# travelingspaceman/LowThrustOpt

Measured on NVIDIA B200. Metric: segment-propagations/s (fp64 state+STM), higher is better.
Workload: dtype f64

## Files before the change

lowthrustopt_b200/csrc/lto_direct_cw.cu:

```cuda
#include "lto_internal.h"
#include "lto_cw_common.cuh"
#include <algorithm>

namespace lto {

namespace cw {

constexpr int NTILE = 2;
constexpr int NSLOT = 2;
constexpr int XW0 = 2;

template <int NS>
struct Cfg {
    static constexpr int NCOL = NS + 3;
    static constexpr int NW = NTILE + NCOL;
    static constexpr int NTHREADS = 32 * NW;
    static constexpr int SVAL = (NS == 7) ? 10 : 6;
    static constexpr int OFF_H = 13 * SVAL;
    static constexpr int OFF_BM = OFF_H + 1;
    static constexpr int STEP_DOUBLES = OFF_BM + ((NS == 7) ? 3 : 0);
    static constexpr size_t REC_BYTES = (size_t)NTILE * NSLOT * STEP_DOUBLES * 32 * sizeof(double);
    static constexpr int NV = 2 * (NS + 3);
    static constexpr size_t OUT_TILE_BYTES = (size_t)16 * NS * NV * sizeof(double);
    static constexpr size_t OUT_BYTES = (size_t)NTILE * OUT_TILE_BYTES;
    static constexpr size_t BAR_OFF = REC_BYTES + OUT_BYTES;
    static constexpr size_t FLAG_OFF = BAR_OFF + (size_t)NTILE * NSLOT * 2 * sizeof(unsigned long long);
    static constexpr size_t SMEM = FLAG_OFF + (size_t)NTILE * NSLOT * sizeof(int);
};

using namespace cwc;

template <int NS, bool PUB = true>
__device__ __forceinline__ double x_step(double (&r)[3], double (&v)[3], double& m, const double (&u)[3], double omega,
                                         double mdot, double h, const EPConst& c, double* __restrict__ rec, double& maxErr) {
    constexpr int SVAL = Cfg<NS>::SVAL;
    const double h2 = h * h;
    const double w2 = 2.0 * omega;
    const double kom6 = c.kthr / c.default_mass;
    double a[13][3];
    double ev[3] = {0.0, 0.0, 0.0}, ea[3] = {0.0, 0.0, 0.0};
    if (PUB) rec[Cfg<NS>::OFF_H * 32] = h;
#pragma unroll
    for (int j = 0; j < 13; ++j) {
        double R[3], V[3];
#pragma unroll
        for (int q = 0; q < 3; ++q) {
            double accv = 0.0, accr = 0.0;
#pragma unroll
            for (int l = 0; l < j; ++l) {
                if (lto_tab::Bf(j, l) != 0.0) accv = fma(lto_tab::Bf(j, l), a[l][q], accv);
                if (lto_tab::Gf(j, l) != 0.0) accr = fma(lto_tab::Gf(j, l), a[l][q], accr);
            }
            V[q] = (j == 0) ? v[q] : fma(h, accv, v[q]);
            R[q] = (j == 0) ? r[q] : fma(h2, accr, fma(h * lto_tab::Cf(j), v[q], r[q]));
        }
        const double dx1 = R[0] + c.mu, dx2 = dx1 - 1.0;
        const double yz = fma(R[1], R[1], R[2] * R[2]);
        const double i1 = fast_rsqrt(fma(dx1, dx1, yz));
        const double i2 = fast_rsqrt(fma(dx2, dx2, yz));
        const double i1s = i1 * i1, i2s = i2 * i2;
        const double a31 = c.m1 * i1s * i1, a32 = c.mu * i2s * i2;
        const double gg1 = 1.0 - (a31 + a32);
        double kom = kom6, im = 0.0;
        if (NS == 7) { im = fast_rcp(fma(h * lto_tab::Cf(j), mdot, m)); kom = c.kthr * im; }
        a[j][0] = fma(u[0], kom, fma(-a31, dx1, fma(-a32, dx2, fma(w2, V[1], R[0]))));
        a[j][1] = fma(u[1], kom, fma(gg1, R[1], -w2 * V[0]));
        a[j][2] = fma(u[2], kom, (gg1 - 1.0) * R[2]);
        if (PUB && j != 10) {
            const double a51 = 3.0 * i1s * a31, a52 = 3.0 * i2s * a32;
            const double s5 = a51 + a52;
            const double p1 = a51 * dx1, p2 = a52 * dx2;
            const double t = p1 + p2;
            const double s5y = s5 * R[1];
            double* w = rec + j * SVAL * 32;
            w[0 * 32] = fma(p1, dx1, fma(p2, dx2, gg1));
            w[1 * 32] = fma(s5y, R[1], gg1);
            w[2 * 32] = fma(s5 * R[2], R[2], gg1 - 1.0);
            w[3 * 32] = t * R[1];
            w[4 * 32] = t * R[2];
            w[5 * 32] = s5y * R[2];
            if (NS == 7) {
                w[6 * 32] = kom;
                const double k2 = -kom * im;
#pragma unroll
                for (int q = 0; q < 3; ++q) w[(7 + q) * 32] = k2 * u[q];
            }
        }
        if (lto_tab::PSIf(j) != 0.0) {
#pragma unroll
            for (int q = 0; q < 3; ++q) { ev[q] = fma(lto_tab::PSIf(j), V[q], ev[q]); ea[q] = fma(lto_tab::PSIf(j), a[j][q], ea[q]); }
        }
    }
    double delta = 0.0;
#pragma unroll
    for (int q = 0; q < 3; ++q) {
        double sv = 0.0, sr = 0.0;
#pragma unroll
        for (int l = 0; l < 13; ++l) {
            if (lto_tab::CHIf(l) != 0.0) sv = fma(lto_tab::CHIf(l), a[l][q], sv);
            if (lto_tab::CHIBf(l) != 0.0) sr = fma(lto_tab::CHIBf(l), a[l][q], sr);
        }
        r[q] = fma(h2, sr, fma(h, v[q], r[q]));
        v[q] = fma(h, sv, v[q]);
        delta = fmax(delta, fmax(fabs(ev[q]), fabs(ea[q])));
    }
    if (NS == 7) m = fma(h, mdot, m);
    delta *= fabs(h * lto_tab::ERRC);
    maxErr = fmax(maxErr, delta);
    return delta;
}

template <int NS>
__device__ __forceinline__ void col_step(double (&sr)[3], double (&sv)[3], double& sm, double bm, const double (&ec)[3],
                                         double omega, double kom6, const double* __restrict__ rec) {
    constexpr int SVAL = Cfg<NS>::SVAL;
    constexpr bool MASS = (NS == 7);
    const double h = rec[Cfg<NS>::OFF_H * 32];
    const double h2 = h * h;
    const double w2 = 2.0 * omega;
    double a[13][3];
#pragma unroll
    for (int j = 0; j < 13; ++j) {
        if (j == 10) continue;
        double R[3], V[3];
#pragma unroll
        for (int q = 0; q < 3; ++q) {
            double accv = 0.0, accr = 0.0;
#pragma unroll
            for (int l = 0; l < j; ++l) {
                if (lto_tab::Bf(j, l) != 0.0) accv = fma(lto_tab::Bf(j, l), a[l][q], accv);
                if (lto_tab::Gf(j, l) != 0.0) accr = fma(lto_tab::Gf(j, l), a[l][q], accr);
            }
            V[q] = (j == 0) ? sv[q] : fma(h, accv, sv[q]);
            R[q] = (j == 0) ? sr[q] : fma(h2, accr, fma(h * lto_tab::Cf(j), sv[q], sr[q]));
        }
        const double* w = rec + j * SVAL * 32;
        double U[6];
#pragma unroll
        for (int q = 0; q < 6; ++q) U[q] = w[q * 32];
        const double kom = MASS ? w[6 * 32] : kom6;
        double acc[3];
        acc[0] = fma(ec[0], kom, w2 * V[1]);
        acc[1] = fma(ec[1], kom, -w2 * V[0]);
        acc[2] = ec[2] * kom;
        if (MASS) {
            const double smj = fma(h * lto_tab::Cf(j), bm, sm);
#pragma unroll
            for (int q = 0; q < 3; ++q) acc[q] = fma(w[(7 + q) * 32], smj, acc[q]);
        }
        sym3_mul_acc(U, R, acc);
#pragma unroll
        for (int q = 0; q < 3; ++q) a[j][q] = acc[q];
    }
#pragma unroll
    for (int q = 0; q < 3; ++q) {
        double dv = 0.0, dr = 0.0;
#pragma unroll
        for (int l = 0; l < 13; ++l) {
            if (lto_tab::CHIf(l) != 0.0) dv = fma(lto_tab::CHIf(l), a[l][q], dv);
            if (lto_tab::CHIBf(l) != 0.0) dr = fma(lto_tab::CHIBf(l), a[l][q], dr);
        }
        sr[q] = fma(h2, dr, fma(h, sv[q], sr[q]));
        sv[q] = fma(h, dv, sv[q]);
    }
    if (MASS) sm = fma(h, bm, sm);
}

struct ColState { double sr[3], sv[3], sm, bm; };

template <int NS>
__device__ __forceinline__ void col_init(ColState& c, int col) {
#pragma unroll
    for (int q = 0; q < 3; ++q) { c.sr[q] = (col == q) ? 1.0 : 0.0; c.sv[q] = (col == q + 3) ? 1.0 : 0.0; }
    c.sm = (NS == 7 && col == 6) ? 1.0 : 0.0;
    c.bm = 0.0;
}

template <int NS>
__device__ __forceinline__ void col_store(double* __restrict__ stage, const ColState& c, int col, int lane) {
    constexpr int NV = 2 * (NS + 3);
    const int back = lane & 1, gc = col - NS;
    const int ocol = (gc >= 0) ? (2 * NS + (back ? 3 : 0) + gc) : ((back ? NS : 0) + col);
    double* J = stage + (lane >> 1) * (NS * NV) + ocol * NS;
    const double rj = (col >= 3 && col < 6) ? -1.0 : 1.0;
    const double sp = back ? -rj : 1.0;
    const double sq = back ? rj : 1.0;
    J[0] = sp * c.sr[0]; J[1] = sp * c.sr[1]; J[2] = sp * c.sr[2];
    J[3] = sq * c.sv[0]; J[4] = sq * c.sv[1]; J[5] = sq * c.sv[2];
    if (NS == 7) J[6] = sp * c.sm;
}

template <int NS>
__device__ __forceinline__ void column_warp(const DirectArgs& a, long long n_tiles, int col, int lane, double* recs, double* outs, unsigned bars) {
    typedef Cfg<NS> C;
    const int nstep = a.cfg.nsteps - 1;
    const double omega = (lane & 1) ? -1.0 : 1.0;
    const double kom6 = a.c.kthr / a.c.default_mass;
    const int gc = col - NS;
    const double ec[3] = {gc == 0 ? 1.0 : 0.0, gc == 1 ? 1.0 : 0.0, gc == 2 ? 1.0 : 0.0};
    ColState cs[NTILE];
    unsigned g = 0;
    for (long long pair = blockIdx.x; pair * NTILE < n_tiles; pair += gridDim.x) {
#pragma unroll
        for (int t = 0; t < NTILE; ++t) col_init<NS>(cs[t], col);
        for (int k = 0; k < nstep; ++k, ++g) {
            const unsigned slot = g & (NSLOT - 1), par = (g / NSLOT) & 1;
#ifndef LTO_K1_NO_PACE
            asm volatile("bar.sync 3, %0;" ::"n"(32 * C::NCOL) : "memory");
#endif
#pragma unroll
            for (int t = 0; t < NTILE; ++t) {
                const double* rec = recs + (size_t)(t * NSLOT + slot) * C::STEP_DOUBLES * 32 + lane;
                const unsigned full = bars + (unsigned)((t * NSLOT + slot) * 16), empty = full + 8;
                mbar_wait(full, par);
                if (NS == 7 && k == 0 && gc >= 0) cs[t].bm = rec[(C::OFF_BM + gc) * 32];
                col_step<NS>(cs[t].sr, cs[t].sv, cs[t].sm, cs[t].bm, ec, omega, kom6, rec);
                mbar_arrive(empty);
                if (k == nstep - 1) {
                    const long long tile = pair * NTILE + t;
                    const long long seg0 = tile * 16;
                    double* stage = outs + (size_t)t * (C::OUT_TILE_BYTES / sizeof(double));
                    const bool leader = (col == 0 && lane == 0);
                    if (leader) bulk_store_wait_read_but<NTILE - 1>();
                    asm volatile("bar.sync 2, %0;" ::"n"(32 * C::NCOL) : "memory");
                    col_store<NS>(stage, cs[t], col, lane);
                    fence_proxy_async();
                    asm volatile("bar.sync 2, %0;" ::"n"(32 * C::NCOL) : "memory");
                    if (leader && seg0 < a.n_seg) {
                        const long long nseg = (a.n_seg - seg0 < 16) ? (a.n_seg - seg0) : 16;
                        bulk_store(a.jac + seg0 * (long long)(NS * C::NV), smem_u32(stage), (unsigned)(nseg * NS * C::NV * sizeof(double)));
                    }
                }
            }
        }
    }
    if (col == 0 && lane == 0) bulk_store_wait_all();
}

template <int NS>
__device__ __forceinline__ void state_warp(const DirectArgs& a, long long n_tiles, int t, int lane, double* recs, unsigned bars) {
    typedef Cfg<NS> C;
    const int nsteps = a.cfg.nsteps, nstep = nsteps - 1;
    const int back = lane & 1;
    const double omega = back ? -1.0 : 1.0;
    double r[3], v[3], m = a.c.default_mass, u[3], bm[3] = {0.0, 0.0, 0.0}, mdot = 0.0, t0 = 0.0, t1 = 1.0, maxErr = 0.0;
    unsigned g = 0;
    for (long long pair = blockIdx.x; pair * NTILE < n_tiles; pair += gridDim.x) {
        const long long seg = (pair * NTILE + t) * 16 + (lane >> 1);
        {
            const long long sc = seg < a.n_seg ? seg : a.n_seg - 1;
            const long long ia = lto_node_a(sc, a.npt);
            const double* X = (back ? a.Xb : a.Xa) + ia * NS;
            const double* U = (back ? a.ub : a.ua) + ia * 3;
            r[0] = X[0]; r[1] = X[1]; r[2] = X[2];
            v[0] = X[3]; v[1] = X[4]; v[2] = X[5];
            if (back) { v[0] = -v[0]; v[1] = -v[1]; v[2] = -v[2]; }
            if (NS == 7) m = X[6];
            u[0] = U[0]; u[1] = U[1]; u[2] = U[2];
            const double ta = a.ta[ia], tb = a.tb[ia];
            t0 = ta; t1 = ta + (tb - ta) / 2.0;
            const double un = sqrt(fma(u[0], u[0], fma(u[1], u[1], u[2] * u[2])));
            mdot = -omega * un * a.c.cmdot;
            if (NS == 7) {
#pragma unroll
                for (int q = 0; q < 3; ++q) {
                    const double uh = (un > 0.0) ? u[q] / un : 1.0;
                    bm[q] = -omega * a.c.cmdot * uh;
                }
            }
            maxErr = 0.0;
        }
        for (int k = 0; k < nstep; ++k, ++g) {
            const unsigned slot = g & (NSLOT - 1), use = g / NSLOT;
            double* rec = recs + (size_t)(t * NSLOT + slot) * C::STEP_DOUBLES * 32 + lane;
            const unsigned full = bars + (unsigned)((t * NSLOT + slot) * 16), empty = full + 8;
            if (use > 0) mbar_wait(empty, (use - 1) & 1);
            const double h = linrange_at(t0, t1, nsteps, k + 1) - linrange_at(t0, t1, nsteps, k);
            if (NS == 7) {
#pragma unroll
                for (int q = 0; q < 3; ++q) rec[(C::OFF_BM + q) * 32] = bm[q];
            }
            x_step<NS>(r, v, m, u, omega, mdot, h, a.c, rec, maxErr);
            mbar_arrive(full);
        }
        const unsigned fullmask = 0xffffffffu;
        double xe[NS];
        xe[0] = r[0]; xe[1] = r[1]; xe[2] = r[2];
        xe[3] = back ? -v[0] : v[0]; xe[4] = back ? -v[1] : v[1]; xe[5] = back ? -v[2] : v[2];
        if (NS == 7) xe[6] = m;
        bool bad = false;
#pragma unroll
        for (int q = 0; q < NS; ++q) {
            const double other = __shfl_xor_sync(fullmask, xe[q], 1);
            const double d = xe[q] - other;
            bad |= !(d == d);
            if (!back && seg < a.n_seg) a.defect[seg * NS + q] = d;
        }
        const double me_o = __shfl_xor_sync(fullmask, maxErr, 1);
        if (!back && seg < a.n_seg) {
            if (a.errors) a.errors[seg] = fmax(maxErr, me_o);
            if (a.status) a.status[seg] = bad ? LTO_ST_NAN : LTO_OK;
        }
    }
}


template <int NS>
__device__ __forceinline__ void state_warp_adapt(const DirectArgs& a, long long n_tiles, int t, int lane, double* recs, unsigned bars, volatile int* lastf) {
    typedef Cfg<NS> C;
    const int back = lane & 1;
    const double omega = back ? -1.0 : 1.0;
    const unsigned fullmask = 0xffffffffu;
    double r[3], v[3], m = a.c.default_mass, u[3], bm[3] = {0.0, 0.0, 0.0}, mdot = 0.0, dummy = 0.0;
    unsigned g = 0;
    for (long long pair = blockIdx.x; pair * NTILE < n_tiles; pair += gridDim.x) {
        const long long seg = (pair * NTILE + t) * 16 + (lane >> 1);
        const long long sc = seg < a.n_seg ? seg : a.n_seg - 1;
        const long long ia = lto_node_a(sc, a.npt);
        const double* X = (back ? a.Xb : a.Xa) + ia * NS;
        const double* U = (back ? a.ub : a.ua) + ia * 3;
        r[0] = X[0]; r[1] = X[1]; r[2] = X[2];
        v[0] = X[3]; v[1] = X[4]; v[2] = X[5];
        if (back) { v[0] = -v[0]; v[1] = -v[1]; v[2] = -v[2]; }
        if (NS == 7) m = X[6];
        u[0] = U[0]; u[1] = U[1]; u[2] = U[2];
        const double ta = a.ta[ia], tb = a.tb[ia];
        const double t0 = ta, tfinal = ta + (tb - ta) / 2.0;
        const double un = sqrt(fma(u[0], u[0], fma(u[1], u[1], u[2] * u[2])));
        mdot = -omega * un * a.c.cmdot;
        if (NS == 7) {
#pragma unroll
            for (int q = 0; q < 3; ++q) { const double uh = (un > 0.0) ? u[q] / un : 1.0; bm[q] = -omega * a.c.cmdot * uh; }
        }
        const double hmax = (tfinal - t0) / 2.5, hmin = (tfinal - t0) / 1e7;
        double tt = t0, h = (tfinal - t0) / 50.0;
        int status = 0, nt = 0;
        bool done = !((tt < tfinal) && (h >= hmin));
        while (true) {
            const unsigned slot = g & (NSLOT - 1), use = g / NSLOT;
            double* rec = recs + (size_t)(t * NSLOT + slot) * C::STEP_DOUBLES * 32 + lane;
            const unsigned full = bars + (unsigned)((t * NSLOT + slot) * 16), empty = full + 8;
            if (use > 0) mbar_wait(empty, (use - 1) & 1);
            if (NS == 7) {
#pragma unroll
                for (int q = 0; q < 3; ++q) rec[(C::OFF_BM + q) * 32] = bm[q];
            }
            bool pending = !done;
            if (done) {
#pragma unroll
                for (int j = 0; j < 13 * C::SVAL; ++j) rec[j * 32] = 0.0;
                rec[C::OFF_H * 32] = 0.0;
            }
            while (__any_sync(fullmask, pending)) {
                if (pending) {
                    if (tt + h > tfinal) h = tfinal - tt;
                    if (nt >= a.cfg.max_attempts) { status = LTO_ST_MAXSTEPS; done = true; pending = false; }
                }
                if (pending) {
                    ++nt;
                    double r2[3] = {r[0], r[1], r[2]}, v2[3] = {v[0], v[1], v[2]}, m2 = m;
                    const double xn = fmax(fmax(fmax(fabs(r[0]), fabs(r[1])), fmax(fabs(r[2]), fabs(v[0]))), fmax(fmax(fabs(v[1]), fabs(v[2])), NS == 7 ? fabs(m) : 0.0));
                    double delta = x_step<NS>(r2, v2, m2, u, omega, mdot, h, a.c, rec, dummy);
                    if (!(delta == delta)) { status = LTO_ST_NAN; done = true; pending = false; }
                    else {
                        const double tau = a.cfg.tol * fmax(xn, 1.0);
                        if (delta <= tau) {
                            tt += h;
                            r[0] = r2[0]; r[1] = r2[1]; r[2] = r2[2]; v[0] = v2[0]; v[1] = v2[1]; v[2] = v2[2]; m = m2;
                            pending = false;
                        }
                        if (delta == 0.0) delta = 1e-16;
                        h = fmin(hmax, 0.8 * h * pow(tau / delta, 0.125));
                        if (!((tt < tfinal) && (h >= hmin))) { done = true; if (pending) { status = LTO_ST_HMIN; pending = false; } }
                    }
                }
            }
            if (status != 0) {
#pragma unroll
                for (int j = 0; j < 13 * C::SVAL; ++j) rec[j * 32] = 0.0;
                rec[C::OFF_H * 32] = 0.0;
            }
            const bool all_done = __all_sync(fullmask, done);
            if (lane == 0) lastf[t * NSLOT + slot] = all_done ? 1 : 0;
            mbar_arrive(full);
            ++g;
            if (all_done) break;
        }
        if (status == 0 && tt < tfinal) status = LTO_ST_HMIN;
        double xe[NS];
        xe[0] = r[0]; xe[1] = r[1]; xe[2] = r[2];
        xe[3] = back ? -v[0] : v[0]; xe[4] = back ? -v[1] : v[1]; xe[5] = back ? -v[2] : v[2];
        if (NS == 7) xe[6] = m;
        bool bad = false;
#pragma unroll
        for (int q = 0; q < NS; ++q) {
            const double other = __shfl_xor_sync(fullmask, xe[q], 1);
            const double d = xe[q] - other;
            bad |= !(d == d);
            if (!back && seg < a.n_seg) a.defect[seg * NS + q] = d;
        }
        const int st_o = __shfl_xor_sync(fullmask, status, 1);
        if (!back && seg < a.n_seg) {
            if (a.errors) a.errors[seg] = 0.0;
            if (a.status) a.status[seg] = status ? status : (st_o ? st_o : (bad ? LTO_ST_NAN : LTO_OK));
        }
    }
}

template <int NS>
__device__ __forceinline__ void column_warp_adapt(const DirectArgs& a, long long n_tiles, int col, int lane, double* recs, double* outs, unsigned bars,
                                                  volatile int* lastf) {
    typedef Cfg<NS> C;
    const double omega = (lane & 1) ? -1.0 : 1.0;
    const double kom6 = a.c.kthr / a.c.default_mass;
    const int gc = col - NS;
    const double ec[3] = {gc == 0 ? 1.0 : 0.0, gc == 1 ? 1.0 : 0.0, gc == 2 ? 1.0 : 0.0};
    ColState cs[NTILE];
    unsigned g[NTILE];
#pragma unroll
    for (int t = 0; t < NTILE; ++t) g[t] = 0;
    for (long long pair = blockIdx.x; pair * NTILE < n_tiles; pair += gridDim.x) {
#pragma unroll
        for (int t = 0; t < NTILE; ++t) col_init<NS>(cs[t], col);
        unsigned alive = (1u << NTILE) - 1u, first = alive;
        while (alive) {
#ifndef LTO_K1_NO_PACE
            asm volatile("bar.sync 3, %0;" ::"n"(32 * C::NCOL) : "memory");
#endif
#pragma unroll
            for (int t = 0; t < NTILE; ++t) {
                if (!(alive & (1u << t))) continue;
                const unsigned slot = g[t] & (NSLOT - 1), par = (g[t] / NSLOT) & 1;
                const double* rec = recs + (size_t)(t * NSLOT + slot) * C::STEP_DOUBLES * 32 + lane;
                const unsigned full = bars + (unsigned)((t * NSLOT + slot) * 16), empty = full + 8;
                mbar_wait(full, par);
                if (NS == 7 && (first & (1u << t)) && gc >= 0) cs[t].bm = rec[(C::OFF_BM + gc) * 32];
                first &= ~(1u << t);
                const bool last = lastf[t * NSLOT + slot] != 0;
                col_step<NS>(cs[t].sr, cs[t].sv, cs[t].sm, cs[t].bm, ec, omega, kom6, rec);
                mbar_arrive(empty);
                ++g[t];
                if (last) alive &= ~(1u << t);
            }
        }
#pragma unroll
        for (int t = 0; t < NTILE; ++t) {
            const long long tile = pair * NTILE + t;
            const long long seg0 = tile * 16;
            double* stage = outs + (size_t)t * (C::OUT_TILE_BYTES / sizeof(double));
            const bool leader = (col == 0 && lane == 0);
            if (leader) bulk_store_wait_read_but<NTILE - 1>();
            asm volatile("bar.sync 2, %0;" ::"n"(32 * C::NCOL) : "memory");
            col_store<NS>(stage, cs[t], col, lane);
            fence_proxy_async();
            asm volatile("bar.sync 2, %0;" ::"n"(32 * C::NCOL) : "memory");
            if (leader && seg0 < a.n_seg) {
                const long long nseg = (a.n_seg - seg0 < 16) ? (a.n_seg - seg0) : 16;
                bulk_store(a.jac + seg0 * (long long)(NS * C::NV), smem_u32(stage), (unsigned)(nseg * NS * C::NV * sizeof(double)));
            }
        }
    }
    if (col == 0 && lane == 0) bulk_store_wait_all();
}

template <int NS, bool ADAPT>
__global__ void __launch_bounds__(Cfg<NS>::NTHREADS, 1) k_direct_cw(DirectArgs a, long long n_tiles) {
    typedef Cfg<NS> C;
    extern __shared__ __align__(16) unsigned char smem_raw[];
    double* recs = reinterpret_cast<double*>(smem_raw);
    double* outs = reinterpret_cast<double*>(smem_raw + C::REC_BYTES);
    const unsigned bars = smem_u32(smem_raw + C::BAR_OFF);
    const int warp = threadIdx.x >> 5, lane = threadIdx.x & 31;
    if (threadIdx.x == 0) {
#pragma unroll
        for (int i = 0; i < NTILE * NSLOT; ++i) {
            mbar_init(bars + i * 16, 32);
            mbar_init(bars + i * 16 + 8, 32 * C::NCOL);
        }
    }
    __syncthreads();
    volatile int* lastf = reinterpret_cast<volatile int*>(smem_raw + C::FLAG_OFF);
    if (warp >= XW0 && warp < XW0 + NTILE) {
        if (ADAPT) state_warp_adapt<NS>(a, n_tiles, warp - XW0, lane, recs, bars, lastf);
        else state_warp<NS>(a, n_tiles, warp - XW0, lane, recs, bars);
    } else {
        const int col = warp < XW0 ? warp : warp - NTILE;
        if (ADAPT) column_warp_adapt<NS>(a, n_tiles, col, lane, recs, outs, bars, lastf);
        else column_warp<NS>(a, n_tiles, col, lane, recs, outs, bars);
    }
}

template <int NS>
__global__ void __launch_bounds__(128) k_direct_state(DirectArgs a) {
    const int nsteps = a.cfg.nsteps, nstep = nsteps - 1;
    const int lane = threadIdx.x & 31, back = lane & 1;
    const double omega = back ? -1.0 : 1.0;
    const long long n_pairs32 = (a.n_seg + 15) / 16;
    const long long warp0 = ((long long)blockIdx.x * blockDim.x + threadIdx.x) >> 5, nwarp = ((long long)gridDim.x * blockDim.x) >> 5;
    for (long long w = warp0; w < n_pairs32; w += nwarp) {
        const long long seg = w * 16 + (lane >> 1);
        const long long sc = seg < a.n_seg ? seg : a.n_seg - 1;
        const long long ia = lto_node_a(sc, a.npt);
        const double* X = (back ? a.Xb : a.Xa) + ia * NS;
        const double* U = (back ? a.ub : a.ua) + ia * 3;
        double r[3] = {X[0], X[1], X[2]}, v[3] = {X[3], X[4], X[5]}, m = a.c.default_mass, u[3] = {U[0], U[1], U[2]}, maxErr = 0.0;
        if (back) { v[0] = -v[0]; v[1] = -v[1]; v[2] = -v[2]; }
        if (NS == 7) m = X[6];
        const double ta = a.ta[ia], tb = a.tb[ia];
        const double t0 = ta, t1 = ta + (tb - ta) / 2.0;
        const double un = sqrt(fma(u[0], u[0], fma(u[1], u[1], u[2] * u[2])));
        const double mdot = -omega * un * a.c.cmdot;
        for (int k = 0; k < nstep; ++k) {
            const double h = linrange_at(t0, t1, nsteps, k + 1) - linrange_at(t0, t1, nsteps, k);
            x_step<NS, false>(r, v, m, u, omega, mdot, h, a.c, nullptr, maxErr);
        }
        const unsigned fullmask = 0xffffffffu;
        double xe[NS];
        xe[0] = r[0]; xe[1] = r[1]; xe[2] = r[2];
        xe[3] = back ? -v[0] : v[0]; xe[4] = back ? -v[1] : v[1]; xe[5] = back ? -v[2] : v[2];
        if (NS == 7) xe[6] = m;
        bool bad = false;
#pragma unroll
        for (int q = 0; q < NS; ++q) {
            const double other = __shfl_xor_sync(fullmask, xe[q], 1);
            const double d = xe[q] - other;
            bad |= !(d == d);
            if (!back && seg < a.n_seg) a.defect[seg * NS + q] = d;
        }
        const double me_o = __shfl_xor_sync(fullmask, maxErr, 1);
        if (!back && seg < a.n_seg) {
            if (a.errors) a.errors[seg] = fmax(maxErr, me_o);
            if (a.status) a.status[seg] = bad ? LTO_ST_NAN : LTO_OK;
        }
    }
}

}

template <int NS>
static cudaError_t launch_state(const DirectArgs& a, cudaStream_t st) {
    int dev = 0, n_sm = 0;
    cudaError_t e = cudaGetDevice(&dev); if (e != cudaSuccess) return e;
    e = cudaDeviceGetAttribute(&n_sm, cudaDevAttrMultiProcessorCount, dev); if (e != cudaSuccess) return e;
    const long long n_warps = (a.n_seg + 15) / 16;
    const long long blocks = (n_warps + 3) / 4;
    const int grid = (int)std::min<long long>(blocks, (long long)n_sm * 16);
    cw::k_direct_state<NS><<<grid, 128, 0, st>>>(a);
    return cudaGetLastError();
}

template <int NS, bool ADAPT>
static cudaError_t launch_cw(const DirectArgs& a, cudaStream_t st) {
    typedef cw::Cfg<NS> C;
    static int n_sm_dev[64] = {0};
    static bool attr_dev[64] = {false};
    int dev = 0;
    { cudaError_t e = cudaGetDevice(&dev); if (e != cudaSuccess) return e; }
    if (dev < 0 || dev >= 64) return cudaErrorInvalidDevice;
    if (!attr_dev[dev]) {
        cudaError_t e = cudaDeviceGetAttribute(&n_sm_dev[dev], cudaDevAttrMultiProcessorCount, dev); if (e != cudaSuccess) return e;
        e = cudaFuncSetAttribute(cw::k_direct_cw<NS, ADAPT>, cudaFuncAttributeMaxDynamicSharedMemorySize, (int)C::SMEM);
        if (e != cudaSuccess) return e;
        attr_dev[dev] = true;
    }
    const int n_sm = n_sm_dev[dev];
    const long long n_tiles = (a.n_seg + 15) / 16;
    const long long n_pairs = (n_tiles + cw::NTILE - 1) / cw::NTILE;
    const int grid = (int)std::min<long long>(n_pairs, (long long)n_sm);
    cw::k_direct_cw<NS, ADAPT><<<grid, C::NTHREADS, C::SMEM, st>>>(a, n_tiles);
    return cudaGetLastError();
}

cudaError_t launch_direct_cw(const DirectArgs& a, int nstate, cudaStream_t st, int* n_launch) {
    *n_launch = 0;
    if (a.n_seg <= 0 || a.n_seg > (1ll << 34)) return cudaErrorNotSupported;
    if (a.cfg.mode != 0 && (a.cfg.err_norm != 0 || a.jac == nullptr)) return cudaErrorNotSupported;
    if (a.jac != nullptr && (reinterpret_cast<uintptr_t>(a.jac) & 15u) != 0) return cudaErrorNotSupported;
    cudaError_t e;
    if (a.jac == nullptr) {
        if (nstate == 7) e = launch_state<7>(a, st);
        else if (nstate == 6) e = launch_state<6>(a, st);
        else return cudaErrorNotSupported;
    } else if (a.cfg.mode != 0) {
        if (nstate == 7) e = launch_cw<7, true>(a, st);
        else if (nstate == 6) e = launch_cw<6, true>(a, st);
        else return cudaErrorNotSupported;
    } else if (nstate == 7) e = launch_cw<7, false>(a, st);
    else if (nstate == 6) e = launch_cw<6, false>(a, st);
    else return cudaErrorNotSupported;
    if (e == cudaSuccess) *n_launch = 1;
    return e;
}

}
```

Measured before the change: 95.63 million.

## Vectorize step records, park column state in shared memory, add profiling hooks

Per-lane step records are now written as contiguous double2 runs instead of a 32-stride layout, so producer stores and column-warp loads become 16-byte vector accesses. Column warps no longer keep per-tile state in registers; they park and unpark it in a new shared-memory region each step, with non-unrolled tile loops, aiming to cut register pressure. The ec vector is replaced by compile-time gc selects and bm is reloaded every step. Optional clock64 profiling compiles in under a macro. The contiguous per-lane layout may cause shared-memory bank conflicts, and parking adds shared traffic each step.

```diff
diff --git a/lowthrustopt_b200/csrc/lto_direct_cw.cu b/lowthrustopt_b200/csrc/lto_direct_cw.cu
--- a/lowthrustopt_b200/csrc/lto_direct_cw.cu
+++ b/lowthrustopt_b200/csrc/lto_direct_cw.cu
@@ -25,14 +25,46 @@
     static constexpr size_t OUT_BYTES = (size_t)NTILE * OUT_TILE_BYTES;
     static constexpr size_t BAR_OFF = REC_BYTES + OUT_BYTES;
     static constexpr size_t FLAG_OFF = BAR_OFF + (size_t)NTILE * NSLOT * 2 * sizeof(unsigned long long);
-    static constexpr size_t SMEM = FLAG_OFF + (size_t)NTILE * NSLOT * sizeof(int);
+    static constexpr size_t PARK_OFF = (FLAG_OFF + (size_t)NTILE * NSLOT * sizeof(int) + 15) & ~(size_t)15;
+    static constexpr int NPARK = (NS == 7) ? 7 : 6;
+    static constexpr size_t SMEM = PARK_OFF + (size_t)NTILE * NCOL * NPARK * 32 * sizeof(double);
 };
+
+enum { K1P_WORK, K1P_BAR, K1P_PACE, K1P_STORE, K1P_TOTAL, K1P_STEPS, K1P_N };
+#ifdef LTO_K1_PROF
+constexpr int K1P_MAX_BLOCKS = 1024, K1P_MAX_WARPS = 16;
+__device__ unsigned long long k1_prof[K1P_MAX_BLOCKS * K1P_MAX_WARPS * K1P_N];
+struct K1Prof {
+    long long c[K1P_N], t, t_begin;
+    __device__ __forceinline__ void start() {
+        for (int i = 0; i < K1P_N; ++i) c[i] = 0;
+        t = t_begin = clock64();
+    }
+    __device__ __forceinline__ void mark() { t = clock64(); }
+    __device__ __forceinline__ void add(int i) { const long long n = clock64(); c[i] += n - t; t = n; }
+    __device__ __forceinline__ void step() { ++c[K1P_STEPS]; }
+    __device__ __forceinline__ void flush(int warp, int lane) {
+        c[K1P_TOTAL] = clock64() - t_begin;
+        if (lane == 0 && blockIdx.x < K1P_MAX_BLOCKS)
+            for (int i = 0; i < K1P_N; ++i) k1_prof[((size_t)blockIdx.x * K1P_MAX_WARPS + warp) * K1P_N + i] = (unsigned long long)c[i];
+    }
+};
+#else
+struct K1Prof {
+    __device__ __forceinline__ void start() {}
+    __device__ __forceinline__ void mark() {}
+    __device__ __forceinline__ void add(int) {}
+    __device__ __forceinline__ void step() {}
+    __device__ __forceinline__ void flush(int, int) {}
+};
+#endif
 
 using namespace cwc;
 
 template <int NS, bool PUB = true>
 __device__ __forceinline__ double x_step(double (&r)[3], double (&v)[3], double& m, const double (&u)[3], double omega,
-                                         double mdot, double h, const EPConst& c, double* __restrict__ rec, double& maxErr) {
+                                         double mdot, double h, const EPConst& c, double* __restrict__ rec, double* __restrict__ stg,
+                                         double& maxErr) {
     constexpr int SVAL = Cfg<NS>::SVAL;
     const double h2 = h * h;
     const double w2 = 2.0 * omega;
@@ -72,18 +104,14 @@
             const double p1 = a51 * dx1, p2 = a52 * dx2;
             const double t = p1 + p2;
             const double s5y = s5 * R[1];
-            double* w = rec + j * SVAL * 32;
-            w[0 * 32] = fma(p1, dx1, fma(p2, dx2, gg1));
-            w[1 * 32] = fma(s5y, R[1], gg1);
-            w[2 * 32] = fma(s5 * R[2], R[2], gg1 - 1.0);
-            w[3 * 32] = t * R[1];
-            w[4 * 32] = t * R[2];
-            w[5 * 32] = s5y * R[2];
+            double2* w = reinterpret_cast<double2*>(stg + j * SVAL * 32);
+            w[0] = make_double2(fma(p1, dx1, fma(p2, dx2, gg1)), fma(s5y, R[1], gg1));
+            w[1] = make_double2(fma(s5 * R[2], R[2], gg1 - 1.0), t * R[1]);
+            w[2] = make_double2(t * R[2], s5y * R[2]);
             if (NS == 7) {
-                w[6 * 32] = kom;
                 const double k2 = -kom * im;
-#pragma unroll
-                for (int q = 0; q < 3; ++q) w[(7 + q) * 32] = k2 * u[q];
+                w[3] = make_double2(kom, k2 * u[0]);
+                w[4] = make_double2(k2 * u[1], k2 * u[2]);
             }
         }
         if (lto_tab::PSIf(j) != 0.0) {
@@ -111,8 +139,8 @@
 }
 
 template <int NS>
-__device__ __forceinline__ void col_step(double (&sr)[3], double (&sv)[3], double& sm, double bm, const double (&ec)[3],
-                                         double omega, double kom6, const double* __restrict__ rec) {
+__device__ __forceinline__ void col_step(double (&sr)[3], double (&sv)[3], double& sm, double bm, int gc,
+                                         double omega, double kom6, const double* __restrict__ rec, const double* __restrict__ stg) {
     constexpr int SVAL = Cfg<NS>::SVAL;
     constexpr bool MASS = (NS == 7);
     const double h = rec[Cfg<NS>::OFF_H * 32];
@@ -134,19 +162,21 @@
             V[q] = (j == 0) ? sv[q] : fma(h, accv, sv[q]);
             R[q] = (j == 0) ? sr[q] : fma(h2, accr, fma(h * lto_tab::Cf(j), sv[q], sr[q]));
         }
-        const double* w = rec + j * SVAL * 32;
-        double U[6];
-#pragma unroll
-        for (int q = 0; q < 6; ++q) U[q] = w[q * 32];
-        const double kom = MASS ? w[6 * 32] : kom6;
+        const double2* w = reinterpret_cast<const double2*>(stg + j * SVAL * 32);
+        const double2 w0 = w[0], w1 = w[1], w2v = w[2];
+        const double U[6] = {w0.x, w0.y, w1.x, w1.y, w2v.x, w2v.y};
+        double2 w3 = make_double2(kom6, 0.0), w4 = make_double2(0.0, 0.0);
+        if (MASS) { w3 = w[3]; w4 = w[4]; }
+        const double kom = w3.x;
         double acc[3];
-        acc[0] = fma(ec[0], kom, w2 * V[1]);
-        acc[1] = fma(ec[1], kom, -w2 * V[0]);
-        acc[2] = ec[2] * kom;
+        acc[0] = fma(w2, V[1], gc == 0 ? kom : 0.0);
+        acc[1] = fma(-w2, V[0], gc == 1 ? kom : 0.0);
+        acc[2] = gc == 2 ? kom : 0.0;
         if (MASS) {
             const double smj = fma(h * lto_tab::Cf(j), bm, sm);
-#pragma unroll
-            for (int q = 0; q < 3; ++q) acc[q] = fma(w[(7 + q) * 32], smj, acc[q]);
+            const double am[3] = {w3.y, w4.x, w4.y};
+#pragma unroll
+            for (int q = 0; q < 3; ++q) acc[q] = fma(am[q], smj, acc[q]);
         }
         sym3_mul_acc(U, R, acc);
 #pragma unroll
@@ -166,14 +196,27 @@
     if (MASS) sm = fma(h, bm, sm);
 }
 
-struct ColState { double sr[3], sv[3], sm, bm; };
+struct ColState { double sr[3], sv[3], sm; };
 
 template <int NS>
 __device__ __forceinline__ void col_init(ColState& c, int col) {
 #pragma unroll
     for (int q = 0; q < 3; ++q) { c.sr[q] = (col == q) ? 1.0 : 0.0; c.sv[q] = (col == q + 3) ? 1.0 : 0.0; }
     c.sm = (NS == 7 && col == 6) ? 1.0 : 0.0;
-    c.bm = 0.0;
+}
+
+template <int NS>
+__device__ __forceinline__ void col_park(double* __restrict__ p, const ColState& c) {
+#pragma unroll
+    for (int q = 0; q < 3; ++q) { p[q * 32] = c.sr[q]; p[(3 + q) * 32] = c.sv[q]; }
+    if (NS == 7) p[6 * 32] = c.sm;
+}
+
+template <int NS>
+__device__ __forceinline__ void col_unpark(const double* __restrict__ p, ColState& c) {
+#pragma unroll
+    for (int q = 0; q < 3; ++q) { c.sr[q] = p[q * 32]; c.sv[q] = p[(3 + q) * 32]; }
+    c.sm = (NS == 7) ? p[6 * 32] : 0.0;
 }
 
 template <int NS>
@@ -191,59 +234,95 @@
 }
 
 template <int NS>
-__device__ __forceinline__ void column_warp(const DirectArgs& a, long long n_tiles, int col, int lane, double* recs, double* outs, unsigned bars) {
+__device__ __forceinline__ double* col_park_at(double* parks, int t, int col, int lane) {
+    return parks + (size_t)(t * Cfg<NS>::NCOL + col) * Cfg<NS>::NPARK * 32 + lane;
+}
+
+template <int NS, bool ADAPT>
+__device__ __forceinline__ bool col_tile_step(int t, unsigned g, int col, int gc, int lane, double omega, double kom6, double* recs, double* parks,
+                                              unsigned bars, volatile int* lastf, K1Prof& pf) {
+    typedef Cfg<NS> C;
+    const unsigned slot = g & (NSLOT - 1), par = (g / NSLOT) & 1;
+    const double* slotp = recs + (size_t)(t * NSLOT + slot) * C::STEP_DOUBLES * 32;
+    const double* rec = slotp + lane;
+    const unsigned full = bars + (unsigned)((t * NSLOT + slot) * 16), empty = full + 8;
+    mbar_wait(full, par);
+    pf.add(K1P_BAR);
+    double* park = col_park_at<NS>(parks, t, col, lane);
+    ColState cs;
+    col_unpark<NS>(park, cs);
+    const double bm = (NS == 7 && gc >= 0) ? rec[(C::OFF_BM + gc) * 32] : 0.0;
+    const bool last = ADAPT && lastf[t * NSLOT + slot] != 0;
+    col_step<NS>(cs.sr, cs.sv, cs.sm, bm, gc, omega, kom6, rec, slotp + lane * C::SVAL);
+    mbar_arrive(empty);
+    col_park<NS>(park, cs);
+    pf.add(K1P_WORK);
+    pf.step();
+    return last;
+}
+
+template <int NS>
+__device__ __forceinline__ void col_tiles_store(const DirectArgs& a, long long pair, int col, int lane, double* outs, double* parks) {
+    typedef Cfg<NS> C;
+    const bool leader = (col == 0 && lane == 0);
+#pragma unroll 1
+    for (int t = 0; t < NTILE; ++t) {
+        const long long seg0 = (pair * NTILE + t) * 16;
+        double* stage = outs + (size_t)t * (C::OUT_TILE_BYTES / sizeof(double));
+        if (leader) bulk_store_wait_read_but<NTILE - 1>();
+        asm volatile("bar.sync 2, %0;" ::"n"(32 * C::NCOL) : "memory");
+        ColState cs;
+        col_unpark<NS>(col_park_at<NS>(parks, t, col, lane), cs);
+        col_store<NS>(stage, cs, col, lane);
+        fence_proxy_async();
+        asm volatile("bar.sync 2, %0;" ::"n"(32 * C::NCOL) : "memory");
+        if (leader && seg0 < a.n_seg) {
+            const long long nseg = (a.n_seg - seg0 < 16) ? (a.n_seg - seg0) : 16;
+            bulk_store(a.jac + seg0 * (long long)(NS * C::NV), smem_u32(stage), (unsigned)(nseg * NS * C::NV * sizeof(double)));
+        }
+    }
+}
+
+template <int NS>
+__device__ __forceinline__ void column_warp(const DirectArgs& a, long long n_tiles, int warp, int col, int lane, double* recs, double* outs, double* parks,
+                                            unsigned bars) {
     typedef Cfg<NS> C;
     const int nstep = a.cfg.nsteps - 1;
     const double omega = (lane & 1) ? -1.0 : 1.0;
     const double kom6 = a.c.kthr / a.c.default_mass;
     const int gc = col - NS;
-    const double ec[3] = {gc == 0 ? 1.0 : 0.0, gc == 1 ? 1.0 : 0.0, gc == 2 ? 1.0 : 0.0};
-    ColState cs[NTILE];
+    K1Prof pf;
+    pf.start();
     unsigned g = 0;
     for (long long pair = blockIdx.x; pair * NTILE < n_tiles; pair += gridDim.x) {
-#pragma unroll
-        for (int t = 0; t < NTILE; ++t) col_init<NS>(cs[t], col);
+#pragma unroll 1
+        for (int t = 0; t < NTILE; ++t) { ColState c; col_init<NS>(c, col); col_park<NS>(col_park_at<NS>(parks, t, col, lane), c); }
         for (int k = 0; k < nstep; ++k, ++g) {
-            const unsigned slot = g & (NSLOT - 1), par = (g / NSLOT) & 1;
+            pf.mark();
 #ifndef LTO_K1_NO_PACE
             asm volatile("bar.sync 3, %0;" ::"n"(32 * C::NCOL) : "memory");
 #endif
-#pragma unroll
-            for (int t = 0; t < NTILE; ++t) {
-                const double* rec = recs + (size_t)(t * NSLOT + slot) * C::STEP_DOUBLES * 32 + lane;
-                const unsigned full = bars + (unsigned)((t * NSLOT + slot) * 16), empty = full + 8;
-                mbar_wait(full, par);
-                if (NS == 7 && k == 0 && gc >= 0) cs[t].bm = rec[(C::OFF_BM + gc) * 32];
-                col_step<NS>(cs[t].sr, cs[t].sv, cs[t].sm, cs[t].bm, ec, omega, kom6, rec);
-                mbar_arrive(empty);
-                if (k == nstep - 1) {
-                    const long long tile = pair * NTILE + t;
-                    const long long seg0 = tile * 16;
-                    double* stage = outs + (size_t)t * (C::OUT_TILE_BYTES / sizeof(double));
-                    const bool leader = (col == 0 && lane == 0);
-                    if (leader) bulk_store_wait_read_but<NTILE - 1>();
-                    asm volatile("bar.sync 2, %0;" ::"n"(32 * C::NCOL) : "memory");
-                    col_store<NS>(stage, cs[t], col, lane);
-                    fence_proxy_async();
-                    asm volatile("bar.sync 2, %0;" ::"n"(32 * C::NCOL) : "memory");
-                    if (leader && seg0 < a.n_seg) {
-                        const long long nseg = (a.n_seg - seg0 < 16) ? (a.n_seg - seg0) : 16;
-                        bulk_store(a.jac + seg0 * (long long)(NS * C::NV), smem_u32(stage), (unsigned)(nseg * NS * C::NV * sizeof(double)));
-                    }
-                }
-            }
-        }
+            pf.add(K1P_PACE);
+#pragma unroll 1
+            for (int t = 0; t < NTILE; ++t) col_tile_step<NS, false>(t, g, col, gc, lane, omega, kom6, recs, parks, bars, nullptr, pf);
+        }
+        pf.mark();
+        col_tiles_store<NS>(a, pair, col, lane, outs, parks);
+        pf.add(K1P_STORE);
     }
     if (col == 0 && lane == 0) bulk_store_wait_all();
-}
-
-template <int NS>
-__device__ __forceinline__ void state_warp(const DirectArgs& a, long long n_tiles, int t, int lane, double* recs, unsigned bars) {
+    pf.flush(warp, lane);
+}
+
+template <int NS>
+__device__ __forceinline__ void state_warp(const DirectArgs& a, long long n_tiles, int warp, int t, int lane, double* recs, unsigned bars) {
     typedef Cfg<NS> C;
     const int nsteps = a.cfg.nsteps, nstep = nsteps - 1;
     const int back = lane & 1;
     const double omega = back ? -1.0 : 1.0;
     double r[3], v[3], m = a.c.default_mass, u[3], bm[3] = {0.0, 0.0, 0.0}, mdot = 0.0, t0 = 0.0, t1 = 1.0, maxErr = 0.0;
+    K1Prof pf;
+    pf.start();
     unsigned g = 0;
     for (long long pair = blockIdx.x; pair * NTILE < n_tiles; pair += gridDim.x) {
         const long long seg = (pair * NTILE + t) * 16 + (lane >> 1);
@@ -272,16 +351,21 @@
         }
         for (int k = 0; k < nstep; ++k, ++g) {
             const unsigned slot = g & (NSLOT - 1), use = g / NSLOT;
-            double* rec = recs + (size_t)(t * NSLOT + slot) * C::STEP_DOUBLES * 32 + lane;
+            double* slotp = recs + (size_t)(t * NSLOT + slot) * C::STEP_DOUBLES * 32;
+            double* rec = slotp + lane;
             const unsigned full = bars + (unsigned)((t * NSLOT + slot) * 16), empty = full + 8;
+            pf.mark();
             if (use > 0) mbar_wait(empty, (use - 1) & 1);
+            pf.add(K1P_BAR);
             const double h = linrange_at(t0, t1, nsteps, k + 1) - linrange_at(t0, t1, nsteps, k);
             if (NS == 7) {
 #pragma unroll
                 for (int q = 0; q < 3; ++q) rec[(C::OFF_BM + q) * 32] = bm[q];
             }
-            x_step<NS>(r, v, m, u, omega, mdot, h, a.c, rec, maxErr);
+            x_step<NS>(r, v, m, u, omega, mdot, h, a.c, rec, slotp + lane * C::SVAL, maxErr);
             mbar_arrive(full);
+            pf.add(K1P_WORK);
+            pf.step();
         }
         const unsigned fullmask = 0xffffffffu;
         double xe[NS];
@@ -302,8 +386,21 @@
             if (a.status) a.status[seg] = bad ? LTO_ST_NAN : LTO_OK;
         }
     }
-}
-
+    pf.flush(warp, lane);
+}
+
+
+template <int NS>
+__device__ __forceinline__ void zero_step_record(double* rec, double* stg) {
+    constexpr int SVAL = Cfg<NS>::SVAL;
+#pragma unroll
+    for (int j = 0; j < 13; ++j) {
+        double2* w = reinterpret_cast<double2*>(stg + j * SVAL * 32);
+#pragma unroll
+        for (int p = 0; p < SVAL / 2; ++p) w[p] = make_double2(0.0, 0.0);
+    }
+    rec[Cfg<NS>::OFF_H * 32] = 0.0;
+}
 
 template <int NS>
 __device__ __forceinline__ void state_warp_adapt(const DirectArgs& a, long long n_tiles, int t, int lane, double* recs, unsigned bars, volatile int* lastf) {
@@ -338,7 +435,9 @@
         bool done = !((tt < tfinal) && (h >= hmin));
         while (true) {
             const unsigned slot = g & (NSLOT - 1), use = g / NSLOT;
-            double* rec = recs + (size_t)(t * NSLOT + slot) * C::STEP_DOUBLES * 32 + lane;
+            double* slotp = recs + (size_t)(t * NSLOT + slot) * C::STEP_DOUBLES * 32;
+            double* rec = slotp + lane;
+            double* stg = slotp + lane * C::SVAL;
             const unsigned full = bars + (unsigned)((t * NSLOT + slot) * 16), empty = full + 8;
             if (use > 0) mbar_wait(empty, (use - 1) & 1);
             if (NS == 7) {
@@ -347,9 +446,7 @@
             }
             bool pending = !done;
             if (done) {
-#pragma unroll
-                for (int j = 0; j < 13 * C::SVAL; ++j) rec[j * 32] = 0.0;
-                rec[C::OFF_H * 32] = 0.0;
+                zero_step_record<NS>(rec, stg);
             }
             while (__any_sync(fullmask, pending)) {
                 if (pending) {
@@ -360,7 +457,7 @@
                     ++nt;
                     double r2[3] = {r[0], r[1], r[2]}, v2[3] = {v[0], v[1], v[2]}, m2 = m;
                     const double xn = fmax(fmax(fmax(fabs(r[0]), fabs(r[1])), fmax(fabs(r[2]), fabs(v[0]))), fmax(fmax(fabs(v[1]), fabs(v[2])), NS == 7 ? fabs(m) : 0.0));
-                    double delta = x_step<NS>(r2, v2, m2, u, omega, mdot, h, a.c, rec, dummy);
+                    double delta = x_step<NS>(r2, v2, m2, u, omega, mdot, h, a.c, rec, stg, dummy);
                     if (!(delta == delta)) { status = LTO_ST_NAN; done = true; pending = false; }
                     else {
                         const double tau = a.cfg.tol * fmax(xn, 1.0);
@@ -375,11 +472,7 @@
                     }
                 }
             }
-            if (status != 0) {
-#pragma unroll
-                for (int j = 0; j < 13 * C::SVAL; ++j) rec[j * 32] = 0.0;
-                rec[C::OFF_H * 32] = 0.0;
-            }
+            if (status != 0) zero_step_record<NS>(rec, stg);
             const bool all_done = __all_sync(fullmask, done);
             if (lane == 0) lastf[t * NSLOT + slot] = all_done ? 1 : 0;
             mbar_arrive(full);
@@ -408,59 +501,39 @@
 }
 
 template <int NS>
-__device__ __forceinline__ void column_warp_adapt(const DirectArgs& a, long long n_tiles, int col, int lane, double* recs, double* outs, unsigned bars,
-                                                  volatile int* lastf) {
-    typedef Cfg<NS> C;
+__device__ __forceinline__ void column_warp_adapt(const DirectArgs& a, long long n_tiles, int warp, int col, int lane, double* recs, double* outs,
+                                                  double* parks, unsigned bars, volatile int* lastf) {
     const double omega = (lane & 1) ? -1.0 : 1.0;
     const double kom6 = a.c.kthr / a.c.default_mass;
     const int gc = col - NS;
-    const double ec[3] = {gc == 0 ? 1.0 : 0.0, gc == 1 ? 1.0 : 0.0, gc == 2 ? 1.0 : 0.0};
-    ColState cs[NTILE];
+    K1Prof pf;
+    pf.start();
     unsigned g[NTILE];
 #pragma unroll
     for (int t = 0; t < NTILE; ++t) g[t] = 0;
     for (long long pair = blockIdx.x; pair * NTILE < n_tiles; pair += gridDim.x) {
-#pragma unroll
-        for (int t = 0; t < NTILE; ++t) col_init<NS>(cs[t], col);
-        unsigned alive = (1u << NTILE) - 1u, first = alive;
+#pragma unroll 1
+        for (int t = 0; t < NTILE; ++t) { ColState c; col_init<NS>(c, col); col_park<NS>(col_park_at<NS>(parks, t, col, lane), c); }
+        unsigned alive = (1u << NTILE) - 1u;
         while (alive) {
+            pf.mark();
 #ifndef LTO_K1_NO_PACE
-            asm volatile("bar.sync 3, %0;" ::"n"(32 * C::NCOL) : "memory");
+            asm volatile("bar.sync 3, %0;" ::"n"(32 * Cfg<NS>::NCOL) : "memory");
 #endif
+            pf.add(K1P_PACE);
 #pragma unroll
             for (int t = 0; t < NTILE; ++t) {
                 if (!(alive & (1u << t))) continue;
-                const unsigned slot = g[t] & (NSLOT - 1), par = (g[t] / NSLOT) & 1;
-                const double* rec = recs + (size_t)(t * NSLOT + slot) * C::STEP_DOUBLES * 32 + lane;
-                const unsigned full = bars + (unsigned)((t * NSLOT + slot) * 16), empty = full + 8;
-                mbar_wait(full, par);
-                if (NS == 7 && (first & (1u << t)) && gc >= 0) cs[t].bm = rec[(C::OFF_BM + gc) * 32];
-                first &= ~(1u << t);
-                const bool last = lastf[t * NSLOT + slot] != 0;
-                col_step<NS>(cs[t].sr, cs[t].sv, cs[t].sm, cs[t].bm, ec, omega, kom6, rec);
-                mbar_arrive(empty);
+                if (col_tile_step<NS, true>(t, g[t], col, gc, lane, omega, kom6, recs, parks, bars, lastf, pf)) alive &= ~(1u << t);
                 ++g[t];
-                if (last) alive &= ~(1u << t);
-            }
-        }
-#pragma unroll
-        for (int t = 0; t < NTILE; ++t) {
-            const long long tile = pair * NTILE + t;
-            const long long seg0 = tile * 16;
-            double* stage = outs + (size_t)t * (C::OUT_TILE_BYTES / sizeof(double));
-            const bool leader = (col == 0 && lane == 0);
-            if (leader) bulk_store_wait_read_but<NTILE - 1>();
-            asm volatile("bar.sync 2, %0;" ::"n"(32 * C::NCOL) : "memory");
-            col_store<NS>(stage, cs[t], col, lane);
-            fence_proxy_async();
-            asm volatile("bar.sync 2, %0;" ::"n"(32 * C::NCOL) : "memory");
-            if (leader && seg0 < a.n_seg) {
-                const long long nseg = (a.n_seg - seg0 < 16) ? (a.n_seg - seg0) : 16;
-                bulk_store(a.jac + seg0 * (long long)(NS * C::NV), smem_u32(stage), (unsigned)(nseg * NS * C::NV * sizeof(double)));
-            }
-        }
+            }
+        }
+        pf.mark();
+        col_tiles_store<NS>(a, pair, col, lane, outs, parks);
+        pf.add(K1P_STORE);
     }
     if (col == 0 && lane == 0) bulk_store_wait_all();
+    pf.flush(warp, lane);
 }
 
 template <int NS, bool ADAPT>
@@ -469,6 +542,7 @@
     extern __shared__ __align__(16) unsigned char smem_raw[];
     double* recs = reinterpret_cast<double*>(smem_raw);
     double* outs = reinterpret_cast<double*>(smem_raw + C::REC_BYTES);
+    double* parks = reinterpret_cast<double*>(smem_raw + C::PARK_OFF);
     const unsigned bars = smem_u32(smem_raw + C::BAR_OFF);
     const int warp = threadIdx.x >> 5, lane = threadIdx.x & 31;
     if (threadIdx.x == 0) {
@@ -482,11 +556,11 @@
     volatile int* lastf = reinterpret_cast<volatile int*>(smem_raw + C::FLAG_OFF);
     if (warp >= XW0 && warp < XW0 + NTILE) {
         if (ADAPT) state_warp_adapt<NS>(a, n_tiles, warp - XW0, lane, recs, bars, lastf);
-        else state_warp<NS>(a, n_tiles, warp - XW0, lane, recs, bars);
+        else state_warp<NS>(a, n_tiles, warp, warp - XW0, lane, recs, bars);
     } else {
         const int col = warp < XW0 ? warp : warp - NTILE;
-        if (ADAPT) column_warp_adapt<NS>(a, n_tiles, col, lane, recs, outs, bars, lastf);
-        else column_warp<NS>(a, n_tiles, col, lane, recs, outs, bars);
+        if (ADAPT) column_warp_adapt<NS>(a, n_tiles, warp, col, lane, recs, outs, parks, bars, lastf);
+        else column_warp<NS>(a, n_tiles, warp, col, lane, recs, outs, parks, bars);
     }
 }
 
@@ -512,7 +586,7 @@
         const double mdot = -omega * un * a.c.cmdot;
         for (int k = 0; k < nstep; ++k) {
             const double h = linrange_at(t0, t1, nsteps, k + 1) - linrange_at(t0, t1, nsteps, k);
-            x_step<NS, false>(r, v, m, u, omega, mdot, h, a.c, nullptr, maxErr);
+            x_step<NS, false>(r, v, m, u, omega, mdot, h, a.c, nullptr, nullptr, maxErr);
         }
         const unsigned fullmask = 0xffffffffu;
         double xe[NS];
@@ -570,6 +644,13 @@
     cw::k_direct_cw<NS, ADAPT><<<grid, C::NTHREADS, C::SMEM, st>>>(a, n_tiles);
     return cudaGetLastError();
 }
+
+#ifdef LTO_K1_PROF
+extern "C" int lto_k1_prof_read(unsigned long long* out, int n_words) {
+    const size_t n = std::min<size_t>((size_t)n_words, sizeof(cw::k1_prof) / sizeof(unsigned long long));
+    return (int)cudaMemcpyFromSymbol(out, cw::k1_prof, n * sizeof(unsigned long long));
+}
+#endif
 
 cudaError_t launch_direct_cw(const DirectArgs& a, int nstate, cudaStream_t st, int* n_launch) {
     *n_launch = 0;
```

After: 100.6 million (median of 6 runs). +5.2%, better.
